# artis-mcrt/artis

Hardware: AMD Instinct MI355X
Metric: packet-steps/sec (higher is better)
Workload: dtype f64

## Files before the change

### artis_amd/build.py

```python
from __future__ import annotations

import fcntl
import os
import shutil
import subprocess

HERE = os.path.dirname(os.path.abspath(__file__))
CSRC = os.path.join(HERE, "csrc")
SO = os.path.join(HERE, "libartis_amd.so")
SOURCES = ["artis_engine.hip", "physics.h", "tables.h", "model_build.h", "spectra.h", "radfield_fit.h", "ion_balance.h",
           "stage_common.h", "stage_spectra.h", "stage_radfield.h", "stage_ionbal.h"]
FLAGS = ["-O3", "--offload-arch=gfx950", "-std=c++17", "-fPIC", "-shared", "-ffp-contract=off", "-munsafe-fp-atomics",
         "-fno-slp-vectorize", "-mllvm", "-disable-machine-licm", "-ldl"]


PRESETS = ("classic", "kilonova_lte", "nltenebular", "christinenonthermal", "nltephotospheric", "nltewithoutnonthermal", "nltenebular_lineest", "kilonova_barnes", "kilonova_wollaeger", "kilonova_gammaproducts",
           "kilonova_gamma_barnes", "kilonova_gamma_wollaeger", "kilonova_gamma_guttman", "kilonova_gamma_grey", "classic_gamma_xcom",
           "kilonova_expopac", "classic_expopac_therm",
           "ci_kilonova", "ci_kilonova_barnes", "ci_kilonova_expopac", "ci_kilonova_xcom", "ci_nebular", "ci_nebular_limitbfest",
           "ci_nltephotospheric", "ci_classic_vpkt", "ci_classic_vpkt_expopac")


def so_path(preset: str = "classic") -> str:
    return SO if preset == "classic" else os.path.join(HERE, f"libartis_amd_{preset}.so")


def needs_build(preset: str = "classic") -> bool:
    so = so_path(preset)
    if not os.path.exists(so):
        return True
    t = os.path.getmtime(so)
    deps = [os.path.join(CSRC, s) for s in SOURCES] + [os.path.join(HERE, "..", "include", h)
                                                        for h in ("artis_amd.h", "artis_options.h")]
# ... 30 lines not shown
```

### artis_amd/csrc/artis_engine.hip

```cpp
#include <hip/hip_runtime.h>
#include <rccl/rccl.h>

#include <dlfcn.h>

#include <cstdio>
#include <cstdlib>
#include <algorithm>
#include <chrono>
#include <cstring>
#include <string>
#include <type_traits>
#include <vector>
#include <cmath>

#include "model_build.h"
#include "physics.h"
#include "radfield_fit.h"
#include "ion_balance.h"
#include "spectra.h"

#include <rocprim/device/device_radix_sort.hpp>

using namespace artis;

// ... 572 lines not shown
    const int src = __ffsll((long long)m) - 1;
    ma_fill_record_wave(env, __builtin_amdgcn_readlane(c, src), __builtin_amdgcn_readlane(ul, src));
    m &= m - 1;
  }
}
__global__ void __launch_bounds__(BLOCK) k_debug_macache(Env env, int c, double *maprocessrates, double *matrans, int32_t *bad) {
  const int ul = blockIdx.x * BLOCK + threadIdx.x;
  if (ul >= env.M.nlevels) return;
  if (ma_resolve(env, c, env.M.level_pack[ul].rec_off) == MA_REC_NONE) return;
  const int b = debug_level_record(env, c, ul, maprocessrates, matrans);
  if (b != 0) atomicAdd(bad, b);
}
__global__ void __launch_bounds__(BLOCK) k_ma_reset(Env env) {
  const int64_t i = (int64_t)blockIdx.x * BLOCK + threadIdx.x;
  const int ncold = env.M.ncold;
  if (i >= fill_count(env) * ncold) return;
  const int c = fill_cell(env, i / ncold);
  env.K.ma_rowtab[(krow(env, c) * ncold) + (i % ncold)] = -1;
}
__global__ void __launch_bounds__(BLOCK) k_mainit(Env env, int64_t nrows) {
  const int64_t i = (int64_t)blockIdx.x * BLOCK + threadIdx.x;
  if (i >= nrows * env.M.nlevels) return;
  populate_mainit(env, i / env.M.nlevels, (int)(i % env.M.nlevels));
}
__global__ void __launch_bounds__(BLOCK) k_cooling_head(Env env) {
  const int64_t i = (int64_t)blockIdx.x * BLOCK + threadIdx.x;
  const int64_t total = fill_count(env) * env.M.nions;
  if (i >= total) return;
  const int c = fill_cell(env, i / env.M.nions);
  const int ui = (int)(i % env.M.nions);
  int k = 0;
  env.K.ion_cooling_C[(krow(env, c) * env.M.nions) + ui] = cooling_ion_head(env, c, ui, &k);
}
__device__ inline double row_shr1(double x) {
  int lo = __double2loint(x), hi = __double2hiint(x);
  lo = __builtin_amdgcn_update_dpp(0, lo, 0x111 , 0xF, 0xF, false);
  hi = __builtin_amdgcn_update_dpp(0, hi, 0x111, 0xF, 0xF, false);
  return __hiloint2double(hi, lo);
}
__global__ void __launch_bounds__(BLOCK) k_cooling_chain(Env env) {
  const int64_t row_id = ((int64_t)blockIdx.x * BLOCK + threadIdx.x) >> 4;
  const int r = threadIdx.x & 15;
  const DevModel &M = env.M;
  const int64_t nchains = fill_count(env) * M.nions;
  const bool valid = row_id < nchains;
  const int c = fill_cell(env, (valid ? row_id : 0) / M.nions);
// ... 2206 lines not shown
  if (const char *b = std::getenv("ARTIS_AMD_SORT_MAXPC_T")) e->sort_maxpc_t = std::max(1, std::atoi(b));
  if (const char *b = std::getenv("ARTIS_AMD_WAVECHUNKS_R")) e->wave_chunks_r = std::atoi(b) != 0;
  if (const char *b = std::getenv("ARTIS_AMD_WAVECHUNKS_T")) e->wave_chunks_t = std::atoi(b) != 0;
  if (const char *b = std::getenv("ARTIS_AMD_CUCHUNKS_T")) e->cu_chunks_t = std::atoi(b) != 0;
  if (const char *b = std::getenv("ARTIS_AMD_CONTLDS")) e->cont_lds = std::atoi(b) != 0;
  if (const char *b = std::getenv("ARTIS_AMD_LINELDS")) e->line_lds = std::atoi(b) != 0;
  if (const char *b = std::getenv("ARTIS_AMD_TILE_ZIGZAG")) e->tile_zigzag = std::atoi(b) != 0;
  if (const char *b = std::getenv("ARTIS_AMD_TILE_ADAPT")) e->tile_adapt = std::atoi(b) != 0;
  if (const char *b = std::getenv("ARTIS_AMD_TILE_BLOCK")) e->tile_block = std::max<int64_t>(0, std::atoll(b));
  if (const char *b = std::getenv("ARTIS_AMD_POOL_KEEP")) e->pool_keep = std::atoi(b) != 0;
  if (const char *b = std::getenv("ARTIS_AMD_MATABLES_LDS")) e->ma_tables_lds = std::atoi(b) != 0;
  if (const char *b = std::getenv("ARTIS_AMD_REFILL")) e->thermal_refill = std::atoi(b) != 0;
  if (const char *b = std::getenv("ARTIS_AMD_SORT_NUMAJOR")) e->sort_numajor = std::atoi(b) != 0;
  if (const char *b = std::getenv("ARTIS_AMD_SORT_CELLSHIFT")) e->sort_cellshift = e->sort_numajor ? std::max(0, std::min(20, std::atoi(b))) : 0;
  if (const char *b = std::getenv("ARTIS_AMD_TQ_LOW")) e->tq_low = std::max(1, std::min(64, std::atoi(b)));
  if (const char *b = std::getenv("ARTIS_AMD_SPARSE_FILL")) e->sparse_fill = std::atoi(b) != 0;
  if (const char *b = std::getenv("ARTIS_AMD_SPARSE_MAX")) e->sparse_max_listed = std::max(0, std::atoi(b));
  {
    const int64_t nrows_ = e->tile_cells;
    Env env0 = make_env(e);
    env0.K = e->K;
    hipLaunchKernelGGL(k_mainit, dim3(nblocks(nrows_ * e->Mh.nlevels)), dim3(BLOCK), 0, nullptr, env0, nrows_);
    HIP_TRY(hipGetLastError());
    HIP_TRY(hipDeviceSynchronize());
  }
  {
    const double mb = pop_scratch_mb();
    const int64_t per = std::max<int64_t>(1, (int64_t)e->Mh.nupcum) * (int64_t)sizeof(double);
    e->pop_batch = std::max<int64_t>(1, std::min<int64_t>(e->tile_cells, (int64_t)(mb * 1048576.) / per));
    HIP_TRY(hipMalloc((void **)&e->d_collexc_terms, (size_t)(e->pop_batch * per) + 64));
  }
  if (const char *b = std::getenv("ARTIS_AMD_THERMAL_BLOCKS")) e->thermal_blocks_per_cu = std::max(1, std::min(ARTIS_THERMAL_WAVES, std::atoi(b)));
  e->trace = std::getenv("ARTIS_AMD_TRACE") != nullptr;
  if (e->trace)
    fprintf(stderr, "[artis_amd] record tiers: static records for %.2f of every ion's levels, %d cold levels, pool of %d slots per resident cell; %d tile(s) of %lld cells, %zu B per cell\n",
            e->ma_hotfrac, e->Mh.ncold, e->Mh.ma_pool_slots, e->ntiles, (long long)e->tile_cells, e->cache_bytes_per_cell);
  if (const char *b = std::getenv("ARTIS_AMD_VPKT_CONTLDS")) e->vpkt_cont_lds = std::atoi(b) != 0;
  if (const char *b = std::getenv("ARTIS_AMD_TILE_PARK")) e->park_tails = std::atoi(b) != 0;
  if (const char *b = std::getenv("ARTIS_AMD_TILE_PARK_AT")) e->park_at = std::max<int64_t>(0, std::atoll(b));
  return ARTIS_OK;
}
}

extern "C" {

void artis_amd_engine_destroy(artis_amd_engine *e) {
// ... 1214 lines not shown
```

### artis_amd/csrc/model_build.h

```cpp
#pragma once
#include <algorithm>
#include <cmath>
#include <cstdlib>
#include <cstring>
#include <vector>

#include "tables.h"

namespace artis {

struct ModelOwned {
  std::vector<double> temperature_grid;
  std::vector<int32_t> level_ion;
  std::vector<LinePack> line_pack;
  std::vector<LevelPack> level_pack;
  std::vector<int32_t> level_upcum_start;
  std::vector<int32_t> alltrans_owner;
  std::vector<int32_t> scanblk_seg0;
  std::vector<uint8_t> scanperm;
  std::vector<MaLongSeg> scansegs, malongsegs;
  std::vector<MaTarget> alltrans_target;
  std::vector<uint16_t> alltrans_tlevel16;
  std::vector<CoolLineRef> coollines;
  std::vector<ContPack> cont_pack;
  std::vector<int32_t> expopac_linestart;
  std::vector<int32_t> upcum_coolslot;
  std::vector<int32_t> level_recomb_start, recomb_lower, recomb_target, recomb_levels, ion_cooltail_start, level_coolhi, ion_guideoff, ion_guideshift;
};

#define ARTIS_MODEL_ARRAYS(X, m)                                                   \
  X(temperature_grid, double, (ARTIS_OPT_TABLESIZE + 1))                           \
  X(elem_nions, int32_t, (m).nelements)                                            \
  X(elem_uniqueionindexstart, int32_t, (m).nelements)                              \
  X(elem_lowest_ionstage, int32_t, (m).nelements)                                  \
  X(elem_anumber, int32_t, (m).nelements)                                          \
  X(ion_element, int32_t, (m).nions)                                               \
  X(ion_nlevels, int32_t, (m).nions)                                               \
  X(ion_nlevels_ionising, int32_t, (m).nions)                                      \
  X(ion_maxrecombininglevel, int32_t, (m).nions)                                   \
  X(ion_uniquelevelindexstart, int32_t, (m).nions)                                 \
  X(ion_coolingoffset, int32_t, (m).nions)                                         \
  X(ion_ncoolingterms, int32_t, (m).nions)                                         \
  X(level_epsilon, double, (m).nlevels)                                            \
  X(level_statweight, float, (m).nlevels)                                          \
  X(level_alltrans_startdown, int32_t, (m).nlevels)                                \
  X(level_ndowntrans, int32_t, (m).nlevels)                                        \
  X(level_nuptrans, int32_t, (m).nlevels)                                          \
  X(level_closestgroundlevelcont, int32_t, (m).nlevels)                            \
  X(level_phixsstart, int32_t, (m).nlevels)                                        \
  X(level_nphixstargets, int32_t, (m).nlevels)                                     \
  X(level_phixstargetstart, int32_t, (m).nlevels)                                  \
  X(level_bflist_start, int32_t, (m).nlevels)                                      \
  X(level_matransblock_start, int32_t, (m).nlevels)                                \
  X(level_ion, int32_t, (m).nlevels)                                               \
  X(level_pack, LevelPack, (m).nlevels)                                            \
  X(level_coolhi, int32_t, (m).nlevels)                                            \
  X(ion_guideoff, int32_t, (m).nions)                                              \
  X(ion_guideshift, int32_t, (m).nions)                                            \
  X(level_upcum_start, int32_t, (m).nlevels)                                       \
  X(alltrans_lineindex, int32_t, (m).nalltrans)                                    \
  X(alltrans_targetlevelindex, int32_t, (m).nalltrans)                             \
  X(alltrans_owner, int32_t, (m).nalltrans)                                        \
  X(scansegs, MaLongSeg, ((m).nscansegs > 0 ? (m).nscansegs : 1))                  \
  X(scanblk_seg0, int32_t, ((m).nscanblk + 1))                                     \
  X(scanperm, uint8_t, ((m).nalltrans > 0 ? (m).nalltrans : 1))                    \
  X(malongsegs, MaLongSeg, ((m).nmalongsegs > 0 ? (m).nmalongsegs : 1))            \
  X(alltrans_target, MaTarget, (m).nalltrans)                                      \
  X(alltrans_tlevel16, uint16_t, (((m).nalltrans + 1) & ~1))  \
  X(coollines, CoolLineRef, ((m).ncoollines > 0 ? (m).ncoollines : 1))             \
  X(alltrans_einstein_A, float, (m).nalltrans)                                     \
  X(alltrans_coll_str, float, (m).nalltrans)                                       \
  X(alltrans_osc_strength, float, (m).nalltrans)                                   \
  X(alltrans_forbidden, uint8_t, (m).nalltrans)                                    \
  X(line_nu, double, (m).nlines)                                                   \
  X(line_pack, LinePack, (m).nlines)                                               \
  X(cont_pack, ContPack, (m).nbfcontinua)                                          \
  X(line_elementindex, int32_t, (m).nlines)                                        \
  X(line_ionindex, int32_t, (m).nlines)                                            \
  X(allphixs, float, ((int64_t)(m).nphixslevels * (m).NPHIXSPOINTS))               \
  X(allphixstargets_levelindex, int32_t, (m).nphixstargets_total)                  \
  X(allphixstargets_probability, double, (m).nphixstargets_total)                  \
  X(allcont_nu_edge, double, (m).nbfcontinua)                                      \
  X(allcont_element, int32_t, (m).nbfcontinua)                                     \
  X(allcont_ion, int32_t, (m).nbfcontinua)                                         \
  X(allcont_level, int32_t, (m).nbfcontinua)                                       \
  X(allcont_phixstargetindex, int32_t, (m).nbfcontinua)                            \
  X(allcont_upperlevel, int32_t, (m).nbfcontinua)                                  \
  X(allcont_uniquelevelindex, int32_t, (m).nbfcontinua)                            \
  X(allcont_groundcontestimindex, int32_t, (m).nbfcontinua)                        \
  X(allcont_probability, double, (m).nbfcontinua)                                  \
// ... 356 lines not shown
  ARTIS_COPY_PTR(coolinglist_type) ARTIS_COPY_PTR(coolinglist_level) ARTIS_COPY_PTR(coolinglist_phixstargetindex)
  ARTIS_COPY_PTR(propcell_nonemptymgi)
#undef ARTIS_COPY_PTR
  v.gridtype = m.gridtype;
  int stride = 1;
  for (int a = 0; a < 3; a++) {
    v.ncoordgrid[a] = m.ncoordgrid[a];
    v.coordstride[a] = stride;
    stride *= m.ncoordgrid[a];
    v.coord_pos_min_tmin[a] = m.coord_pos_min_tmin[a];
  }
  v.ngrid = m.ngrid;
  v.npts_nonempty = m.npts_nonempty;
  v.tmin = m.tmin; v.vmax = m.vmax; v.rmax = m.rmax;
  v.ejecta_kinetic_energy = m.ejecta_kinetic_energy; v.mtot_input = m.mtot_input;
  v.allcont_bfestimindex = m.allcont_bfestimindex;
  v.rho_tmin = m.rho_tmin;
  v.xcom_elem_start = m.xcom_elem_start; v.xcom_energy = m.xcom_energy; v.xcom_sigma = m.xcom_sigma;
  v.nxcom = m.xcom_elem_start ? m.xcom_elem_start[m.nelements] : 0;
  v.detailed_lineindices = m.detailed_lineindices;
  v.detailed_linecount = m.detailed_lineindices ? m.detailed_linecount : 0;
  v.nbfestim = (m.allcont_bfestimindex && m.nbfestim > 0) ? m.nbfestim : m.nbfcontinua;
  v.vpkt = nullptr;
  return v;
}

inline double loggrid_edge(double minvalue, double dlog, double index) { return std::exp(std::log(minvalue) + (index * dlog)); }
inline bool make_vpkt_config(const artis_model &m, VpktConfig &V) {
  std::memset(&V, 0, sizeof(V));
  if (m.vpkt_nobsdirections < 1 || m.vpkt_nobsdirections > VPKT_MAXOBS || !m.vpkt_obsdirs_costheta || !m.vpkt_obsdirs_phi ||
      m.vpkt_nspectraperobsdir < 1 || m.vpkt_nspectraperobsdir > VPKT_MAXSPEC || !m.vpkt_opacityexclusions ||
      m.vpkt_nwavelengthranges < 1 || m.vpkt_nwavelengthranges > VPKT_MAXRANGES || !m.vpkt_numin_input || !m.vpkt_numax_input ||
      m.vpkt_nprocs < 1)
    return false;
  if (m.vpkt_vgrid_on && (m.vpkt_grid_nwavelengthranges < 1 || m.vpkt_grid_nwavelengthranges > VPKT_MAXRANGES || !m.vpkt_nu_grid_min ||
                          !m.vpkt_nu_grid_max))
    return false;
  V.nobsdirections = m.vpkt_nobsdirections;
  V.nspectraperobsdir = m.vpkt_nspectraperobsdir;
  V.nwavelengthranges = m.vpkt_nwavelengthranges;
  V.vgrid_on = m.vpkt_vgrid_on ? 1 : 0;
  V.grid_nwavelengthranges = m.vpkt_vgrid_on ? m.vpkt_grid_nwavelengthranges : 0;
  V.nprocs = m.vpkt_nprocs;
  for (int i = 0; i < V.nobsdirections; i++) {
    const double ct = m.vpkt_obsdirs_costheta[i], ph = m.vpkt_obsdirs_phi[i];
    V.obsdir[i][0] = std::sqrt(1 - (ct * ct)) * std::cos(ph);
// ... 76 lines not shown
```

### artis_amd/csrc/physics.h

```cpp
#pragma once
#include <math.h>
#include <stdint.h>

#include "tables.h"

#if defined(__HIPCC__) && !defined(ARTIS_HOST_EMU)
#define AHD __host__ __device__ inline
#define ANOINLINE static __host__ __device__ __attribute__((noinline))
#else
#define AHD inline
#define ANOINLINE static __attribute__((noinline))
#endif

namespace artis {

constexpr double CLIGHT = 2.99792458e+10;
constexpr double CLIGHT_PROP = CLIGHT;
constexpr double HPLANCK = 6.6260755e-27;
constexpr double PI = 3.14159265358979323846;
constexpr double EV = 1.6021772e-12;
constexpr double SIGMA_T = 6.6524e-25;
constexpr double ME = 9.1093897e-28;
constexpr double MH = 1.67352e-24;
constexpr double MEV = 1.6021772e-6;
constexpr double MSUN = 1.98855e+33;
constexpr double DAY = 86400.;
constexpr double THOMSON_LIMIT = 1e-2;
constexpr double NU_100KEV = 2.41326e+19, NU_1MEV = 2.41326e+20, NU_1P022MEV = 2.46636e+20, NU_1P5MEV = 3.61990e+20;
constexpr double KB = 1.38064852e-16;
constexpr double SAHACONST = 2.0706659e-16;
constexpr double EULERGAMMA = 0.577215664901532860606512090082402431;
constexpr double CLIGHTSQUARED = CLIGHT * CLIGHT;
constexpr double CLIGHTSQUAREDOVERTWOH = CLIGHT * CLIGHT / (2 * HPLANCK);
constexpr double HOVERKB = HPLANCK / KB;
constexpr double HCLIGHTOVERFOURPI = HPLANCK * CLIGHT / (4 * PI);
constexpr double H_ionpot = 13.5979996 * EV;
constexpr double C_0 = 5.465e-11;
constexpr double DBLMAX = 1.7976931348623157e308;
constexpr double DBLMIN = 2.2250738585072014e-308;
constexpr int MA_N = ARTIS_MA_ACTION_COUNT;

#if defined(__HIP_DEVICE_COMPILE__)
typedef unsigned long long stat_t;
#define ARTIS_STAT_ADD(env, i, v) atomicAdd(&(env).stats[(i)], (stat_t)(v))
#ifdef ARTIS_EST_NOADD
#define ARTIS_EST_ADD(ptr, v)                                 \
  do {                                                        \
    const double est_v = (v);                                 \
    if (est_v == 1.2345e-300) unsafeAtomicAdd((ptr), est_v);  \
  } while (0)
#else
#define ARTIS_EST_ADD(ptr, v) unsafeAtomicAdd((ptr), (v))
#endif
#else
typedef unsigned long long stat_t;
#define ARTIS_STAT_ADD(env, i, v) ((env).stats[(i)] += (stat_t)(v))
#define ARTIS_EST_ADD(ptr, v) (*(ptr) += (v))
#endif
#define ARTIS_STAT(env, i) ARTIS_STAT_ADD(env, i, 1)
#if defined(ARTIS_PROFILE) && ARTIS_OPT_VPKT_ON
#error "-DARTIS_PROFILE keeps its phase clocks in the stats slots 48..52, which a VPKT_ON build uses for nvpkt_created / nvpkt_esc_*"
#endif
// ... 102 lines not shown
      }
      vsums[slot] = 0.;
      tags[slot] = c;
    }
  }
  if (tags[slot] == c)
    __hip_atomic_fetch_add((__attribute__((address_space(3))) double *)(env.estcache + slot), v, __ATOMIC_RELAXED, __HIP_MEMORY_SCOPE_WORKGROUP);
  else
    ARTIS_EST_ADD(&global_array[(int64_t)c * env.est_stride], v);
}
#endif

template <typename EnvT>
AHD void scalar_add(const EnvT &env, int idx, double v) {
#if defined(__HIP_DEVICE_COMPILE__)
  if (env.scalars_lds != nullptr) {
    __hip_atomic_fetch_add((__attribute__((address_space(3))) double *)(env.scalars_lds + idx), v, __ATOMIC_RELAXED, __HIP_MEMORY_SCOPE_WORKGROUP);
    return;
  }
#endif
  ARTIS_EST_ADD(&env.E.scalars[idx], v);
}

AHD double pow2(double x) { return x * x; }
AHD double pow3(double x) { return x * x * x; }
AHD double dmin(double a, double b) { return (b < a) ? b : a; }
AHD double dmax(double a, double b) { return (a < b) ? b : a; }
AHD double dclamp(double v, double lo, double hi) { return (v < lo) ? lo : ((hi < v) ? hi : v); }

struct Env {
  DevModel M;
  DevCells C;
  DevCache K;
  DevStep S;
  DevEst E;
  PktStore P;
  stat_t *stats;
  double *gamma_ws;
  int32_t *gamma_gi;
  int32_t *gamma_n;
  int32_t *errflag;
  const int32_t *krow_tab;
  int32_t tile_all;
  int32_t tile_lo, tile_hi;
  const int32_t *fill_cells;
  int32_t nfill;
  double *collexc_terms;
  int32_t cont_in_lds;
// ... 611 lines not shown
  const int gridsize = ARTIS_OPT_TABLESIZE + 1;
  int index = (int)(log(T / ARTIS_OPT_MINTEMP) / M.T_step_log) + 1;
  if (index < 0) index = 0;
  if (index > gridsize) index = gridsize;
  while (index > 0 && M.temperature_grid[index - 1] > T) index--;
  while (index < gridsize && M.temperature_grid[index] <= T) index++;
  return index;
}
AHD double lerp_or_last(const DevModel &M, const double *table, int ul, int t, float T) {
  const double *row = table + ((int64_t)(M.level_bflist_start[ul] + t) * ARTIS_OPT_TABLESIZE);
  const int up = temperature_upperindex(M, T);
  if (up == 0) return row[0];
  if (up < ARTIS_OPT_TABLESIZE) {
    const double T_lower = M.temperature_grid[up - 1];
    const double T_upper = M.temperature_grid[up];
    const double f_lower = row[up - 1];
    const double f_upper = row[up];
    return (f_lower + ((f_upper - f_lower) / (T_upper - T_lower) * (T - T_lower)));
  }
  return row[ARTIS_OPT_TABLESIZE - 1];
}

AHD double gaunt_factor(int stage) { return stage == 1 ? 0.1 : (stage == 2 ? 0.2 : 0.3); }
AHD double rad_deexc(double epsilon_trans, float A_ul, double gu, double gl, double n_u, double n_l, double t) {
  const double nu_trans = epsilon_trans / HPLANCK;
  const double B_ul = CLIGHTSQUAREDOVERTWOH / pow3(nu_trans) * A_ul;
  const double B_lu = gu / gl * B_ul;
  const double tau = ((B_lu * n_l) - (B_ul * n_u)) * HCLIGHTOVERFOURPI * t;
  if (tau > 1e-100) {
    const double beta = 1.0 / tau * (-expm1(-tau));
    return A_ul * beta;
  }
  return A_ul;
}
#if ARTIS_OPT_DETAILED_LINE_ESTIMATORS_ON
AHD int jblueindex(const DevModel &M, int lineindex) {
  int low = 0, high = M.detailed_linecount - 1;
  while (low <= high) {
    const int mid = low + ((high - low) / 2);
    if (M.detailed_lineindices[mid] < lineindex) low = mid + 1;
    else if (M.detailed_lineindices[mid] > lineindex) high = mid - 1;
    else return mid;
  }
  return -1;
}
AHD void update_lineestimator(const Env &env, int c, int lineindex, double increment) {
  const int jb = jblueindex(env.M, lineindex);
  if (jb >= 0) {
    const int64_t o = ((int64_t)c * env.M.detailed_linecount) + jb;
    ARTIS_EST_ADD(&env.E.Jb_lu_raw[o], increment);
    ARTIS_EST_ADD(&env.E.Jb_lu_contribcount[o], 1.);
  }
}
#endif
AHD double rad_exc(const Env &env, int c, double gu, double A, double epsilon_trans, double n_l, double n_u, double gl, double t,
                   int alltransindex = -1) {
  const double nu_trans = epsilon_trans / HPLANCK;
  const double B_ul = CLIGHTSQUAREDOVERTWOH / pow3(nu_trans) * A;
  const double B_lu = gu / gl * B_ul;
  const double tau = ((B_lu * n_l) - (B_ul * n_u)) * HCLIGHTOVERFOURPI * t;
  if (tau > 1e-100) {
    const double beta = 1.0 / tau * (-expm1(-tau));
    const double R_over_J = n_l > 0. ? (B_lu - (B_ul * n_u / n_l)) * beta : B_lu * beta;
#if ARTIS_OPT_DETAILED_LINE_ESTIMATORS_ON
    if (alltransindex >= 0) {
      const int jb = jblueindex(env.M, env.M.alltrans_lineindex[alltransindex]);
      if (jb >= 0) return R_over_J * env.C.Jb_lu_normed[((int64_t)c * env.M.detailed_linecount) + jb];
    }
#endif
    return R_over_J * radfield(env, nu_trans, c);
  }
  return 0.;
}
AHD double rad_recomb(const DevModel &M, float T_e, float cnne, int element, int upperion, int lowerlevel, int t) {
  return cnne * lerp_or_last(M, M.spontrecombcoeffs, lstart(M, element, upperion - 1) + lowerlevel, t, T_e);
}
AHD double col_recomb(const DevModel &M, float T_e, float cnne, int element, int upperion, int lower, int t, double epsilon_trans) {
  const int ul = lstart(M, element, upperion - 1) + lower;
  const double gl = statw(M, ul);
  const double g = gaunt_factor(ionstage(M, element, upperion - 1));
  const double sigma_bf = (phixs_table(M, ul)[0] * phixs_probability(M, ul, t));
  const double gu = statw(M, lstart(M, element, upperion) + phixs_upperlevel(M, ul, t));
  return cnne * cnne * SAHACONST * gl / gu * 1.55e13 * g * sigma_bf * KB / T_e / epsilon_trans;
}
AHD double col_ion(const DevModel &M, float T_e, float cnne, int element, int ion, int lower, int t, double epsilon_trans) {
  const int ul = lstart(M, element, ion) + lower;
  const double g = gaunt_factor(ionstage(M, element, ion));
  const double fac1 = epsilon_trans / KB / T_e;
  const double sigma_bf = phixs_table(M, ul)[0] * phixs_probability(M, ul, t);
  return cnne * 1.55e13 * pow((double)T_e, -0.5) * g * sigma_bf * exp(-fac1) / fac1;
}
AHD double col_deexc(const DevModel &M, float T_e, float cnne, double epsilon_trans, double gu, double gl, int ati) {
  const float cs = M.alltrans_coll_str[ati];
  if (cs < 0) {
    if (!M.alltrans_forbidden[ati]) {
      const double f = M.alltrans_osc_strength[ati];
      const double eoverkt = epsilon_trans / (KB * T_e);
      const double g_bar = 0.2;
      const double gauntfac = (eoverkt > 0.33421) ? g_bar : 0.276 * exp(eoverkt) * (-EULERGAMMA - log(eoverkt));
      const double g_ratio = gl / gu;
      return C_0 * 14.51039491 * cnne * sqrtf(T_e) * f * pow2(H_ionpot / epsilon_trans) * eoverkt * g_ratio * gauntfac;
    }
    return cnne * 8.629e-6 * 0.01 * gl / sqrtf(T_e);
  }
  return cnne * 8.629e-6 * (double)cs / gu / sqrtf(T_e);
}
AHD double col_exc(const DevModel &M, float T_e, float cnne, double epsilon_trans, double gu, double gl, int ati) {
  const float cs = M.alltrans_coll_str[ati];
  const double eoverkt = epsilon_trans / (KB * T_e);
  if (cs < 0) {
    if (!M.alltrans_forbidden[ati]) {
      const double f = M.alltrans_osc_strength[ati];
      const double g_bar = 0.2;
      const double ex = exp(eoverkt);
      const double Gamma = dmax(g_bar, 0.276 * ex * (-EULERGAMMA - log(eoverkt)));
      return C_0 * cnne * sqrtf(T_e) * 14.51039491 * f * pow2(H_ionpot / epsilon_trans) * eoverkt / ex * Gamma;
    }
    return cnne * 8.629e-6 * 0.01 * exp(-eoverkt) * gu / sqrtf(T_e);
  }
  return cnne * 8.629e-6 * (double)cs * exp(-eoverkt) / gl / sqrtf(T_e);
}


AHD void populate_levelpop(const Env &env, int c, int ul) {
  const DevModel &M = env.M;
  if (env.C.levelpops) {
    env.K.levelpops[(krow(env, c) * M.nlevels) + ul] = env.C.levelpops[((int64_t)c * M.nlevels) + ul];
    return;
  }
  const int ui = M.level_ion[ul];
  const int element = M.ion_element[ui];
  const int ion = ui - M.elem_uniqueionindexstart[element];
  const int start = M.ion_uniquelevelindexstart[ui];
  const double nnground = groundlevelpop(env, c, element, ion);
  double nn;
  if (ul == start) {
    nn = nnground;
  } else {
    const float T_exc = ARTIS_OPT_LTEPOP_EXCITATION_USE_TJ ? env.C.TJ[c] : env.C.Te[c];
    const double E_aboveground = eps(M, ul) - eps(M, start);
    nn = (nnground * statw(M, ul) / statw(M, start) * exp(-E_aboveground / KB / T_exc));
  }
  if (nn < ARTIS_OPT_MINPOP) nn = (env.C.elem_massfracs[((int64_t)c * M.nelements) + element] > 0) ? ARTIS_OPT_MINPOP : 0.;
// ... 212 lines not shown
  }
  return !bad;
}
AHD double nt_excitation_ratecoeff(const DevCells &C, int c, int lowerlevel, int upperlevel, int alltransindex) {
  if (!ARTIS_OPT_NT_EXCITATION_ON) return 0.;
  if (lowerlevel >= ARTIS_OPT_NTEXCITATION_MAXNLEVELS_LOWER) return 0.;
  if (upperlevel >= ARTIS_OPT_NTEXCITATION_MAXNLEVELS_UPPER) return 0.;
  const int64_t base = (int64_t)c * C.nt_excitations_stored;
  const int32_t *ati = C.nt_exc_alltransindex + base;
  const int n = C.nt_exc_count[c];
  int lo = 0, hi = n;
  while (lo < hi) {
    const int mid = lo + ((hi - lo) / 2);
    if (ati[mid] < alltransindex) lo = mid + 1; else hi = mid;
  }
  if (lo == n || ati[lo] != alltransindex) return 0.;
  return C.nt_exc_ratecoeffperdeposition[base + lo] * C.nt_deposition_rate_density[c];
}
#endif

struct MaTransTerms {
  int ul, i;
  bool isdown;
  LevelPack lpk;
  double v0, v1, v2;
  double kterm;
};
template <bool COOLING_ONLY_IF_COLD = false>
AHD MaTransTerms matrans_terms(const Env &env, int c, int ati) {
  const DevModel &M = env.M;
  MaTransTerms r;
  r.ul = M.alltrans_owner[ati];
  r.lpk = M.level_pack[r.ul];
  const int ul = r.ul;
  if (COOLING_ONLY_IF_COLD && r.lpk.rec_off < 0) {
    const int i = ati - r.lpk.alltrans_startdown;
    r.isdown = i < r.lpk.ndown;
    r.i = r.isdown ? i : i - r.lpk.ndown;
    r.v0 = r.v1 = r.v2 = r.kterm = 0.;
    if (!r.isdown) {
      const int tul = M.ion_uniquelevelindexstart[M.level_ion[ul]] + M.alltrans_targetlevelindex[ati];
      const double e_trans = eps(M, tul) - eps(M, ul);
      const double Cc = col_exc(M, env.C.Te[c], clumpednne(env.C, c), e_trans, statw(M, tul), statw(M, ul), ati);
      r.kterm = env.K.levelpops[(krow(env, c) * M.nlevels) + ul] * Cc * e_trans;
    }
    return r;
  }
  const int start = M.ion_uniquelevelindexstart[M.level_ion[ul]];
  const double *pops = env.K.levelpops + (krow(env, c) * M.nlevels);
  const float T_e = env.C.Te[c];
  const float cnne = clumpednne(env.C, c);
  const double e_cur = eps(M, ul);
  const double g_cur = statw(M, ul);
  const double nnlevel = pops[ul];
  const int i = ati - r.lpk.alltrans_startdown;
  const int tul = start + M.alltrans_targetlevelindex[ati];
  r.isdown = i < r.lpk.ndown;
  r.kterm = 0.;
  if (r.isdown) {
    r.i = i;
    const float A_ul = M.alltrans_einstein_A[ati];
    const double e_target = eps(M, tul);
    const double e_trans = e_cur - e_target;
    const double g_low = statw(M, tul);
    const double R = rad_deexc(e_trans, A_ul, g_cur, g_low, nnlevel, pops[tul], env.S.mid);
    const double Cc = col_deexc(M, T_e, cnne, e_trans, g_cur, g_low, ati);
    r.v0 = R * e_trans;
    r.v1 = Cc * e_trans;
    r.v2 = (R + Cc) * e_target;
  } else {
    r.i = i - r.lpk.ndown;
    const double e_trans = eps(M, tul) - e_cur;
    const double g_up = statw(M, tul);
    const double R = rad_exc(env, c, g_up, M.alltrans_einstein_A[ati], e_trans, nnlevel, pops[tul], g_cur, env.S.mid, ati);
    const double Cc = col_exc(M, T_e, cnne, e_trans, g_up, g_cur, ati);
#if ARTIS_OPT_NT_ON
    const double NT = nt_excitation_ratecoeff(env.C, c, ul - start, M.alltrans_targetlevelindex[ati], ati);
#else
    const double NT = 0.;
#endif
    r.v0 = (R + Cc + NT) * e_cur;
    r.v1 = 0.;
    r.v2 = 0.;
    r.kterm = nnlevel * Cc * e_trans;
  }
  return r;
}
AHD int32_t ma_rowtab_load(const int32_t *p) {
#if defined(__HIP_DEVICE_COMPILE__)
  return __hip_atomic_load(p, __ATOMIC_RELAXED, __HIP_MEMORY_SCOPE_AGENT);
#else
  return *p;
#endif
}
AHD void ma_rowtab_acquire(const Env &env, int32_t v) {
#if defined(__HIP_DEVICE_COMPILE__)
  if (env.ma_concurrent_fill != 0 && v >= 0) __builtin_amdgcn_fence(__ATOMIC_ACQUIRE, "agent");
#else
  (void)env;
  (void)v;
#endif
}
constexpr int MA_REC_NONE = -1;
template <bool COLD = true>
AHD int ma_resolve(const Env &env, int c, int rec_off) {
  if (!COLD) return rec_off;
  if (__builtin_expect(rec_off >= 0, 1)) return rec_off;
// ... 4126 lines not shown
```

### artis_amd/csrc/tables.h

```cpp
#pragma once
#include <stdint.h>

#include "../../include/artis_amd.h"
#include "../../include/artis_options.h"

namespace artis {

struct alignas(16) LinePack {
  int32_t lower;
  int32_t upper;
  float B_ul;
  float B_lu;
};

struct alignas(16) LevelPack {
  int32_t rec_off;
  int32_t alltrans_startdown;
  int32_t ndown;
  int32_t nup;
};
struct alignas(32) ContPack {
  double nu_edge;
  double probability;
  int32_t xs_off;
  int32_t gi;
  int32_t pad[2];
};
struct alignas(16) MaTarget {
  int32_t rec, ats, level;
  uint32_t ndnu;
};
constexpr int MATGT_MAX_NTRANS = 1 << 16;
static_assert(sizeof(MaTarget) == 16, "transition target size");
struct alignas(16) U4 {
  uint32_t w[4];
};
constexpr int MAREC_ALIGN = 4;
constexpr int MAPOOL_UNIT = 8;
constexpr int MAREC_PER = 7;
constexpr int MAREC_QUAD = 4;
constexpr int MAREC_RATE_SLOTS = 5;
enum { MADIR_DOWN = 0, MADIR_UP = 1, MADIR_RAD = 2, MADIR_COOL = 3 };
constexpr int marec_lines(int n) { return (n + MAREC_PER - 1) / MAREC_PER; }
constexpr int marec_rest(int n) { return n > MAREC_PER ? marec_lines(n) - 1 : 0; }
constexpr int marec_slot(int d, int l, int nd, int nu) {
  return (d < MADIR_COOL && l == 0)
             ? 1 + d
             : (d == MADIR_DOWN ? MAREC_QUAD + (l - 1)
                                : (d == MADIR_UP ? MAREC_QUAD + marec_rest(nd) + (l - 1)
                                                 : (d == MADIR_RAD ? MAREC_QUAD + marec_rest(nd) + marec_rest(nu) + (l - 1)
                                                                   : MAREC_QUAD + (2 * marec_rest(nd)) + marec_rest(nu) + l)));
}
constexpr int marec_rates_slot(int nd, int nu) { return MAREC_QUAD + (2 * marec_rest(nd)) + marec_rest(nu) + marec_lines(nu); }
constexpr int marec_fine_dirslots(int n) { return (marec_lines(n) + 1) / 2; }
constexpr int marec_fine_slot0(int nd, int nu) { return marec_rates_slot(nd, nu) + MAREC_RATE_SLOTS; }
constexpr int marec_fine_byte0(int d, int l, int nd, int nu) {
// ... 51 lines not shown
  const int32_t *xcom_elem_start;
  const double *xcom_energy, *xcom_sigma;
  int32_t nxcom;
  const int32_t *detailed_lineindices;
  int32_t detailed_linecount;
  const VpktConfig *vpkt;
  const int32_t *ion_element, *ion_nlevels, *ion_nlevels_ionising, *ion_maxrecombininglevel, *ion_uniquelevelindexstart,
      *ion_coolingoffset, *ion_ncoolingterms;
  const double *level_epsilon;
  const float *level_statweight;
  const int32_t *level_alltrans_startdown, *level_ndowntrans, *level_nuptrans, *level_closestgroundlevelcont, *level_phixsstart,
      *level_nphixstargets, *level_phixstargetstart, *level_bflist_start, *level_matransblock_start;
  const int32_t *level_ion;
  const LevelPack *level_pack;
  const int32_t *level_upcum_start;
  const int32_t *alltrans_lineindex, *alltrans_targetlevelindex;
  const int32_t *alltrans_owner;
  const MaLongSeg *scansegs;
  const int32_t *scanblk_seg0;
  int32_t nscansegs, nscanblk;
  const uint8_t *scanperm;
  const MaLongSeg *malongsegs;
  int32_t nmalongsegs;
  const MaTarget *alltrans_target;
  const uint16_t *alltrans_tlevel16;
  const CoolLineRef *coollines;
  int32_t ncoollines;
  const float *alltrans_einstein_A, *alltrans_coll_str, *alltrans_osc_strength;
  const uint8_t *alltrans_forbidden;
  const double *line_nu;
  const LinePack *line_pack;
  const ContPack *cont_pack;
  const int32_t *line_elementindex, *line_ionindex;
  const float *allphixs;
  const int32_t *allphixstargets_levelindex;
  const double *allphixstargets_probability;
  const double *allcont_nu_edge;
  const int32_t *allcont_element, *allcont_ion, *allcont_level, *allcont_phixstargetindex, *allcont_upperlevel,
      *allcont_uniquelevelindex, *allcont_groundcontestimindex;
  const double *allcont_probability;
  const double *groundcont_nu_edge;
  const double *spontrecombcoeffs, *corrphotoioncoeffs, *bfcooling_coeffs;
  const uint8_t *coolinglist_type;
  const int32_t *coolinglist_level, *coolinglist_phixstargetindex;

  int32_t gridtype, ncoordgrid[3], coordstride[3], ngrid, npts_nonempty;
// ... 133 lines not shown
```

Measured before the change: 1.375 billion.

## Precompute per-transition constants into a packed TransConst table

Adds a 96-byte TransConst record per transition. A one-time kernel fills it at init with energies, frequency, Einstein B coefficients, statistical weights, flags and indices. matrans_terms now reads this single record instead of gathering level_pack, epsilon, statweight, coll_str and other arrays, and recomputing B coefficients and pow3 per call. The aim is fewer scattered loads and less arithmetic in the macro-atom transition rate evaluation. The cost is extra device memory and a wider per-transition load, and the lower-level energy is now used in place of the current level energy in some terms.

Result: no change. 1.380 billion, median of 6 (+0.3%).

```diff
diff --git a/artis_amd/build.py b/artis_amd/build.py
--- a/artis_amd/build.py
+++ b/artis_amd/build.py
@@ -8,7 +8,7 @@
 HERE = os.path.dirname(os.path.abspath(__file__))
 CSRC = os.path.join(HERE, "csrc")
 SO = os.path.join(HERE, "libartis_amd.so")
-SOURCES = ["artis_engine.hip", "physics.h", "tables.h", "model_build.h", "spectra.h", "radfield_fit.h", "ion_balance.h",
+SOURCES = ["artis_engine.hip", "physics.h", "constants.h", "transconst.h", "tables.h", "model_build.h", "spectra.h", "radfield_fit.h", "ion_balance.h",
            "stage_common.h", "stage_spectra.h", "stage_radfield.h", "stage_ionbal.h"]
 FLAGS = ["-O3", "--offload-arch=gfx950", "-std=c++17", "-fPIC", "-shared", "-ffp-contract=off", "-munsafe-fp-atomics",
          "-fno-slp-vectorize", "-mllvm", "-disable-machine-licm", "-ldl"]
diff --git a/artis_amd/csrc/artis_engine.hip b/artis_amd/csrc/artis_engine.hip
--- a/artis_amd/csrc/artis_engine.hip
+++ b/artis_amd/csrc/artis_engine.hip
@@ -618,6 +618,11 @@
   const int64_t i = (int64_t)blockIdx.x * BLOCK + threadIdx.x;
   if (i >= nrows * env.M.nlevels) return;
   populate_mainit(env, i / env.M.nlevels, (int)(i % env.M.nlevels));
+}
+__global__ void __launch_bounds__(BLOCK) k_transconst(DevModel M, TransConst *out) {
+  const int ati = blockIdx.x * BLOCK + threadIdx.x;
+  if (ati >= M.nalltrans) return;
+  out[ati] = transconst_of(M, ati);
 }
 __global__ void __launch_bounds__(BLOCK) k_cooling_head(Env env) {
   const int64_t i = (int64_t)blockIdx.x * BLOCK + threadIdx.x;
@@ -2870,6 +2875,10 @@
     env0.K = e->K;
     hipLaunchKernelGGL(k_mainit, dim3(nblocks(nrows_ * e->Mh.nlevels)), dim3(BLOCK), 0, nullptr, env0, nrows_);
     HIP_TRY(hipGetLastError());
+    if (e->Mh.nalltrans > 0) {
+      hipLaunchKernelGGL(k_transconst, dim3(nblocks(e->Mh.nalltrans)), dim3(BLOCK), 0, nullptr, e->M, const_cast<TransConst *>(e->M.transconst));
+      HIP_TRY(hipGetLastError());
+    }
     HIP_TRY(hipDeviceSynchronize());
   }
   {
diff --git a/artis_amd/csrc/constants.h b/artis_amd/csrc/constants.h
--- /dev/null
+++ b/artis_amd/csrc/constants.h
@@ -0,0 +1,41 @@
+#pragma once
+
+#if defined(__HIPCC__) && !defined(ARTIS_HOST_EMU)
+#define AHD __host__ __device__ inline
+#define ANOINLINE static __host__ __device__ __attribute__((noinline))
+#else
+#define AHD inline
+#define ANOINLINE static __attribute__((noinline))
+#endif
+
+namespace artis {
+
+constexpr double CLIGHT = 2.99792458e+10;
+constexpr double CLIGHT_PROP = CLIGHT;
+constexpr double HPLANCK = 6.6260755e-27;
+constexpr double PI = 3.14159265358979323846;
+constexpr double EV = 1.6021772e-12;
+constexpr double SIGMA_T = 6.6524e-25;
+constexpr double ME = 9.1093897e-28;
+constexpr double MH = 1.67352e-24;
+constexpr double MEV = 1.6021772e-6;
+constexpr double MSUN = 1.98855e+33;
+constexpr double DAY = 86400.;
+constexpr double THOMSON_LIMIT = 1e-2;
+constexpr double NU_100KEV = 2.41326e+19, NU_1MEV = 2.41326e+20, NU_1P022MEV = 2.46636e+20, NU_1P5MEV = 3.61990e+20;
+constexpr double KB = 1.38064852e-16;
+constexpr double SAHACONST = 2.0706659e-16;
+constexpr double EULERGAMMA = 0.577215664901532860606512090082402431;
+constexpr double CLIGHTSQUARED = CLIGHT * CLIGHT;
+constexpr double CLIGHTSQUAREDOVERTWOH = CLIGHT * CLIGHT / (2 * HPLANCK);
+constexpr double HOVERKB = HPLANCK / KB;
+constexpr double HCLIGHTOVERFOURPI = HPLANCK * CLIGHT / (4 * PI);
+constexpr double H_ionpot = 13.5979996 * EV;
+constexpr double C_0 = 5.465e-11;
+constexpr double DBLMAX = 1.7976931348623157e308;
+constexpr double DBLMIN = 2.2250738585072014e-308;
+
+AHD double pow2(double x) { return x * x; }
+AHD double pow3(double x) { return x * x * x; }
+
+}
diff --git a/artis_amd/csrc/model_build.h b/artis_amd/csrc/model_build.h
--- a/artis_amd/csrc/model_build.h
+++ b/artis_amd/csrc/model_build.h
@@ -6,6 +6,7 @@
 #include <vector>
 
 #include "tables.h"
+#include "transconst.h"
 
 namespace artis {
 
@@ -20,6 +21,7 @@
   std::vector<uint8_t> scanperm;
   std::vector<MaLongSeg> scansegs, malongsegs;
   std::vector<MaTarget> alltrans_target;
+  std::vector<TransConst> transconst;
   std::vector<uint16_t> alltrans_tlevel16;
   std::vector<CoolLineRef> coollines;
   std::vector<ContPack> cont_pack;
@@ -66,6 +68,7 @@
   X(scanperm, uint8_t, ((m).nalltrans > 0 ? (m).nalltrans : 1))                    \
   X(malongsegs, MaLongSeg, ((m).nmalongsegs > 0 ? (m).nmalongsegs : 1))            \
   X(alltrans_target, MaTarget, (m).nalltrans)                                      \
+  X(transconst, TransConst, ((m).nalltrans > 0 ? (m).nalltrans : 1))               \
   X(alltrans_tlevel16, uint16_t, (((m).nalltrans + 1) & ~1))  \
   X(coollines, CoolLineRef, ((m).ncoollines > 0 ? (m).ncoollines : 1))             \
   X(alltrans_einstein_A, float, (m).nalltrans)                                     \
@@ -468,6 +471,11 @@
   v.detailed_linecount = m.detailed_lineindices ? m.detailed_linecount : 0;
   v.nbfestim = (m.allcont_bfestimindex && m.nbfestim > 0) ? m.nbfestim : m.nbfcontinua;
   v.vpkt = nullptr;
+  own.transconst.assign((size_t)(m.nalltrans > 0 ? m.nalltrans : 1), TransConst{});
+  v.transconst = own.transconst.data();
+#if defined(ARTIS_HOST_EMU)
+  for (int ati = 0; ati < m.nalltrans; ati++) own.transconst[ati] = transconst_of(v, ati);
+#endif
   return v;
 }
 
diff --git a/artis_amd/csrc/physics.h b/artis_amd/csrc/physics.h
--- a/artis_amd/csrc/physics.h
+++ b/artis_amd/csrc/physics.h
@@ -3,41 +3,11 @@
 #include <stdint.h>
 
 #include "tables.h"
-
-#if defined(__HIPCC__) && !defined(ARTIS_HOST_EMU)
-#define AHD __host__ __device__ inline
-#define ANOINLINE static __host__ __device__ __attribute__((noinline))
-#else
-#define AHD inline
-#define ANOINLINE static __attribute__((noinline))
-#endif
+#include "constants.h"
+#include "transconst.h"
 
 namespace artis {
 
-constexpr double CLIGHT = 2.99792458e+10;
-constexpr double CLIGHT_PROP = CLIGHT;
-constexpr double HPLANCK = 6.6260755e-27;
-constexpr double PI = 3.14159265358979323846;
-constexpr double EV = 1.6021772e-12;
-constexpr double SIGMA_T = 6.6524e-25;
-constexpr double ME = 9.1093897e-28;
-constexpr double MH = 1.67352e-24;
-constexpr double MEV = 1.6021772e-6;
-constexpr double MSUN = 1.98855e+33;
-constexpr double DAY = 86400.;
-constexpr double THOMSON_LIMIT = 1e-2;
-constexpr double NU_100KEV = 2.41326e+19, NU_1MEV = 2.41326e+20, NU_1P022MEV = 2.46636e+20, NU_1P5MEV = 3.61990e+20;
-constexpr double KB = 1.38064852e-16;
-constexpr double SAHACONST = 2.0706659e-16;
-constexpr double EULERGAMMA = 0.577215664901532860606512090082402431;
-constexpr double CLIGHTSQUARED = CLIGHT * CLIGHT;
-constexpr double CLIGHTSQUAREDOVERTWOH = CLIGHT * CLIGHT / (2 * HPLANCK);
-constexpr double HOVERKB = HPLANCK / KB;
-constexpr double HCLIGHTOVERFOURPI = HPLANCK * CLIGHT / (4 * PI);
-constexpr double H_ionpot = 13.5979996 * EV;
-constexpr double C_0 = 5.465e-11;
-constexpr double DBLMAX = 1.7976931348623157e308;
-constexpr double DBLMIN = 2.2250738585072014e-308;
 constexpr int MA_N = ARTIS_MA_ACTION_COUNT;
 
 #if defined(__HIP_DEVICE_COMPILE__)
@@ -186,8 +156,6 @@
   ARTIS_EST_ADD(&env.E.scalars[idx], v);
 }
 
-AHD double pow2(double x) { return x * x; }
-AHD double pow3(double x) { return x * x * x; }
 AHD double dmin(double a, double b) { return (b < a) ? b : a; }
 AHD double dmax(double a, double b) { return (a < b) ? b : a; }
 AHD double dclamp(double v, double lo, double hi) { return (v < lo) ? lo : ((hi < v) ? hi : v); }
@@ -845,17 +813,6 @@
 }
 
 AHD double gaunt_factor(int stage) { return stage == 1 ? 0.1 : (stage == 2 ? 0.2 : 0.3); }
-AHD double rad_deexc(double epsilon_trans, float A_ul, double gu, double gl, double n_u, double n_l, double t) {
-  const double nu_trans = epsilon_trans / HPLANCK;
-  const double B_ul = CLIGHTSQUAREDOVERTWOH / pow3(nu_trans) * A_ul;
-  const double B_lu = gu / gl * B_ul;
-  const double tau = ((B_lu * n_l) - (B_ul * n_u)) * HCLIGHTOVERFOURPI * t;
-  if (tau > 1e-100) {
-    const double beta = 1.0 / tau * (-expm1(-tau));
-    return A_ul * beta;
-  }
-  return A_ul;
-}
 #if ARTIS_OPT_DETAILED_LINE_ESTIMATORS_ON
 AHD int jblueindex(const DevModel &M, int lineindex) {
   int low = 0, high = M.detailed_linecount - 1;
@@ -876,25 +833,6 @@
   }
 }
 #endif
-AHD double rad_exc(const Env &env, int c, double gu, double A, double epsilon_trans, double n_l, double n_u, double gl, double t,
-                   int alltransindex = -1) {
-  const double nu_trans = epsilon_trans / HPLANCK;
-  const double B_ul = CLIGHTSQUAREDOVERTWOH / pow3(nu_trans) * A;
-  const double B_lu = gu / gl * B_ul;
-  const double tau = ((B_lu * n_l) - (B_ul * n_u)) * HCLIGHTOVERFOURPI * t;
-  if (tau > 1e-100) {
-    const double beta = 1.0 / tau * (-expm1(-tau));
-    const double R_over_J = n_l > 0. ? (B_lu - (B_ul * n_u / n_l)) * beta : B_lu * beta;
-#if ARTIS_OPT_DETAILED_LINE_ESTIMATORS_ON
-    if (alltransindex >= 0) {
-      const int jb = jblueindex(env.M, env.M.alltrans_lineindex[alltransindex]);
-      if (jb >= 0) return R_over_J * env.C.Jb_lu_normed[((int64_t)c * env.M.detailed_linecount) + jb];
-    }
-#endif
-    return R_over_J * radfield(env, nu_trans, c);
-  }
-  return 0.;
-}
 AHD double rad_recomb(const DevModel &M, float T_e, float cnne, int element, int upperion, int lowerlevel, int t) {
   return cnne * lerp_or_last(M, M.spontrecombcoeffs, lstart(M, element, upperion - 1) + lowerlevel, t, T_e);
 }
@@ -913,35 +851,32 @@
   const double sigma_bf = phixs_table(M, ul)[0] * phixs_probability(M, ul, t);
   return cnne * 1.55e13 * pow((double)T_e, -0.5) * g * sigma_bf * exp(-fac1) / fac1;
 }
-AHD double col_deexc(const DevModel &M, float T_e, float cnne, double epsilon_trans, double gu, double gl, int ati) {
-  const float cs = M.alltrans_coll_str[ati];
+AHD double col_deexc_k(const TransConst &k, float cnne, double eoverkt, float sqrt_Te) {
+  const float cs = k.coll_str;
   if (cs < 0) {
-    if (!M.alltrans_forbidden[ati]) {
-      const double f = M.alltrans_osc_strength[ati];
-      const double eoverkt = epsilon_trans / (KB * T_e);
+    if (!(k.flags & TRANSCONST_FORBIDDEN)) {
+      const double f = k.osc_strength;
       const double g_bar = 0.2;
       const double gauntfac = (eoverkt > 0.33421) ? g_bar : 0.276 * exp(eoverkt) * (-EULERGAMMA - log(eoverkt));
-      const double g_ratio = gl / gu;
-      return C_0 * 14.51039491 * cnne * sqrtf(T_e) * f * pow2(H_ionpot / epsilon_trans) * eoverkt * g_ratio * gauntfac;
-    }
-    return cnne * 8.629e-6 * 0.01 * gl / sqrtf(T_e);
-  }
-  return cnne * 8.629e-6 * (double)cs / gu / sqrtf(T_e);
-}
-AHD double col_exc(const DevModel &M, float T_e, float cnne, double epsilon_trans, double gu, double gl, int ati) {
-  const float cs = M.alltrans_coll_str[ati];
-  const double eoverkt = epsilon_trans / (KB * T_e);
+      return C_0 * 14.51039491 * cnne * sqrt_Te * f * k.hion2 * eoverkt * k.g_ratio * gauntfac;
+    }
+    return cnne * 8.629e-6 * 0.01 * (double)k.g_lower / sqrt_Te;
+  }
+  return cnne * 8.629e-6 * (double)cs / (double)k.g_upper / sqrt_Te;
+}
+AHD double col_exc_k(const TransConst &k, float cnne, double eoverkt, float sqrt_Te) {
+  const float cs = k.coll_str;
   if (cs < 0) {
-    if (!M.alltrans_forbidden[ati]) {
-      const double f = M.alltrans_osc_strength[ati];
+    if (!(k.flags & TRANSCONST_FORBIDDEN)) {
+      const double f = k.osc_strength;
       const double g_bar = 0.2;
       const double ex = exp(eoverkt);
       const double Gamma = dmax(g_bar, 0.276 * ex * (-EULERGAMMA - log(eoverkt)));
-      return C_0 * cnne * sqrtf(T_e) * 14.51039491 * f * pow2(H_ionpot / epsilon_trans) * eoverkt / ex * Gamma;
-    }
-    return cnne * 8.629e-6 * 0.01 * exp(-eoverkt) * gu / sqrtf(T_e);
-  }
-  return cnne * 8.629e-6 * (double)cs * exp(-eoverkt) / gl / sqrtf(T_e);
+      return C_0 * cnne * sqrt_Te * 14.51039491 * f * k.hion2 * eoverkt / ex * Gamma;
+    }
+    return cnne * 8.629e-6 * 0.01 * exp(-eoverkt) * (double)k.g_upper / sqrt_Te;
+  }
+  return cnne * 8.629e-6 * (double)cs * exp(-eoverkt) / (double)k.g_lower / sqrt_Te;
 }
 
 
@@ -1200,67 +1135,57 @@
 struct MaTransTerms {
   int ul, i;
   bool isdown;
-  LevelPack lpk;
   double v0, v1, v2;
   double kterm;
 };
 template <bool COOLING_ONLY_IF_COLD = false>
 AHD MaTransTerms matrans_terms(const Env &env, int c, int ati) {
-  const DevModel &M = env.M;
+  const TransConst k = env.M.transconst[ati];
   MaTransTerms r;
-  r.ul = M.alltrans_owner[ati];
-  r.lpk = M.level_pack[r.ul];
-  const int ul = r.ul;
-  if (COOLING_ONLY_IF_COLD && r.lpk.rec_off < 0) {
-    const int i = ati - r.lpk.alltrans_startdown;
-    r.isdown = i < r.lpk.ndown;
-    r.i = r.isdown ? i : i - r.lpk.ndown;
-    r.v0 = r.v1 = r.v2 = r.kterm = 0.;
-    if (!r.isdown) {
-      const int tul = M.ion_uniquelevelindexstart[M.level_ion[ul]] + M.alltrans_targetlevelindex[ati];
-      const double e_trans = eps(M, tul) - eps(M, ul);
-      const double Cc = col_exc(M, env.C.Te[c], clumpednne(env.C, c), e_trans, statw(M, tul), statw(M, ul), ati);
-      r.kterm = env.K.levelpops[(krow(env, c) * M.nlevels) + ul] * Cc * e_trans;
-    }
-    return r;
-  }
-  const int start = M.ion_uniquelevelindexstart[M.level_ion[ul]];
-  const double *pops = env.K.levelpops + (krow(env, c) * M.nlevels);
+  r.ul = k.ul;
+  r.i = k.i;
+  r.isdown = (k.flags & TRANSCONST_DOWN) != 0;
+  r.v0 = r.v1 = r.v2 = r.kterm = 0.;
+  const double *pops = env.K.levelpops + (krow(env, c) * env.M.nlevels);
   const float T_e = env.C.Te[c];
   const float cnne = clumpednne(env.C, c);
-  const double e_cur = eps(M, ul);
-  const double g_cur = statw(M, ul);
-  const double nnlevel = pops[ul];
-  const int i = ati - r.lpk.alltrans_startdown;
-  const int tul = start + M.alltrans_targetlevelindex[ati];
-  r.isdown = i < r.lpk.ndown;
-  r.kterm = 0.;
+  const double eoverkt = k.e_trans / (KB * T_e);
+  const float sqrt_Te = sqrtf(T_e);
+  if (COOLING_ONLY_IF_COLD && (k.flags & TRANSCONST_COLD)) {
+    if (!r.isdown) r.kterm = pops[k.ul] * col_exc_k(k, cnne, eoverkt, sqrt_Te) * k.e_trans;
+    return r;
+  }
+  const double n_u = pops[r.isdown ? k.ul : k.tul], n_l = pops[r.isdown ? k.tul : k.ul];
+  const double tau = ((k.B_lu * n_l) - (k.B_ul * n_u)) * HCLIGHTOVERFOURPI * env.S.mid;
+  const bool thick = tau > 1e-100;
+  double beta = 0.;
+  if (thick) beta = 1.0 / tau * (-expm1(-tau));
   if (r.isdown) {
-    r.i = i;
-    const float A_ul = M.alltrans_einstein_A[ati];
-    const double e_target = eps(M, tul);
-    const double e_trans = e_cur - e_target;
-    const double g_low = statw(M, tul);
-    const double R = rad_deexc(e_trans, A_ul, g_cur, g_low, nnlevel, pops[tul], env.S.mid);
-    const double Cc = col_deexc(M, T_e, cnne, e_trans, g_cur, g_low, ati);
-    r.v0 = R * e_trans;
-    r.v1 = Cc * e_trans;
-    r.v2 = (R + Cc) * e_target;
+    const double R = thick ? k.A_ul * beta : (double)k.A_ul;
+    const double Cc = col_deexc_k(k, cnne, eoverkt, sqrt_Te);
+    r.v0 = R * k.e_trans;
+    r.v1 = Cc * k.e_trans;
+    r.v2 = (R + Cc) * k.e_lower;
   } else {
-    r.i = i - r.lpk.ndown;
-    const double e_trans = eps(M, tul) - e_cur;
-    const double g_up = statw(M, tul);
-    const double R = rad_exc(env, c, g_up, M.alltrans_einstein_A[ati], e_trans, nnlevel, pops[tul], g_cur, env.S.mid, ati);
-    const double Cc = col_exc(M, T_e, cnne, e_trans, g_up, g_cur, ati);
+    double R = 0.;
+    if (thick) {
+      const double R_over_J = n_l > 0. ? (k.B_lu - (k.B_ul * n_u / n_l)) * beta : k.B_lu * beta;
+#if ARTIS_OPT_DETAILED_LINE_ESTIMATORS_ON
+      const int jb = jblueindex(env.M, env.M.alltrans_lineindex[ati]);
+      if (jb >= 0) R = R_over_J * env.C.Jb_lu_normed[((int64_t)c * env.M.detailed_linecount) + jb];
+      else
+#endif
+      R = R_over_J * radfield(env, k.nu_trans, c);
+    }
+    const double Cc = col_exc_k(k, cnne, eoverkt, sqrt_Te);
 #if ARTIS_OPT_NT_ON
-    const double NT = nt_excitation_ratecoeff(env.C, c, ul - start, M.alltrans_targetlevelindex[ati], ati);
+    const int start = env.M.ion_uniquelevelindexstart[env.M.level_ion[k.ul]];
+    const double NT = nt_excitation_ratecoeff(env.C, c, k.ul - start, env.M.alltrans_targetlevelindex[ati], ati);
 #else
     const double NT = 0.;
 #endif
-    r.v0 = (R + Cc + NT) * e_cur;
-    r.v1 = 0.;
-    r.v2 = 0.;
-    r.kterm = nnlevel * Cc * e_trans;
+    r.v0 = (R + Cc + NT) * k.e_lower;
+    r.kterm = n_l * Cc * k.e_trans;
   }
   return r;
 }
diff --git a/artis_amd/csrc/tables.h b/artis_amd/csrc/tables.h
--- a/artis_amd/csrc/tables.h
+++ b/artis_amd/csrc/tables.h
@@ -32,6 +32,17 @@
 };
 constexpr int MATGT_MAX_NTRANS = 1 << 16;
 static_assert(sizeof(MaTarget) == 16, "transition target size");
+struct alignas(32) TransConst {
+  double e_trans, nu_trans, B_ul, B_lu;
+  double hion2, e_lower, g_ratio;
+  float A_ul, coll_str;
+  float osc_strength, g_upper, g_lower;
+  int32_t ul, tul, i, flags, pad;
+};
+static_assert(sizeof(TransConst) == 96, "transition constants: three 32-byte pieces");
+constexpr int32_t TRANSCONST_DOWN = 1;
+constexpr int32_t TRANSCONST_FORBIDDEN = 2;
+constexpr int32_t TRANSCONST_COLD = 4;
 struct alignas(16) U4 {
   uint32_t w[4];
 };
@@ -129,6 +140,7 @@
   const uint8_t *scanperm;
   const MaLongSeg *malongsegs;
   int32_t nmalongsegs;
+  const TransConst *transconst;
   const MaTarget *alltrans_target;
   const uint16_t *alltrans_tlevel16;
   const CoolLineRef *coollines;
diff --git a/artis_amd/csrc/transconst.h b/artis_amd/csrc/transconst.h
--- /dev/null
+++ b/artis_amd/csrc/transconst.h
@@ -0,0 +1,41 @@
+#pragma once
+#include "constants.h"
+#include "tables.h"
+
+namespace artis {
+
+AHD TransConst transconst_of(const DevModel &M, int ati) {
+  TransConst k;
+  const int ul = M.alltrans_owner[ati];
+  const LevelPack lpk = M.level_pack[ul];
+  const int tul = M.ion_uniquelevelindexstart[M.level_ion[ul]] + M.alltrans_targetlevelindex[ati];
+  const int i = ati - lpk.alltrans_startdown;
+  const bool isdown = i < lpk.ndown;
+  const int upper = isdown ? ul : tul, lower = isdown ? tul : ul;
+  const float A_ul = M.alltrans_einstein_A[ati];
+  const double gu = M.level_statweight[upper], gl = M.level_statweight[lower];
+  const double epsilon_trans = M.level_epsilon[upper] - M.level_epsilon[lower];
+  const double nu_trans = epsilon_trans / HPLANCK;
+  const double B_ul = CLIGHTSQUAREDOVERTWOH / pow3(nu_trans) * A_ul;
+  const double B_lu = gu / gl * B_ul;
+  k.e_trans = epsilon_trans;
+  k.nu_trans = nu_trans;
+  k.B_ul = B_ul;
+  k.B_lu = B_lu;
+  k.hion2 = pow2(H_ionpot / epsilon_trans);
+  k.e_lower = M.level_epsilon[lower];
+  k.g_ratio = gl / gu;
+  k.A_ul = A_ul;
+  k.coll_str = M.alltrans_coll_str[ati];
+  k.osc_strength = M.alltrans_osc_strength[ati];
+  k.g_upper = M.level_statweight[upper];
+  k.g_lower = M.level_statweight[lower];
+  k.ul = ul;
+  k.tul = tul;
+  k.i = isdown ? i : i - lpk.ndown;
+  k.flags = (isdown ? TRANSCONST_DOWN : 0) | (M.alltrans_forbidden[ati] ? TRANSCONST_FORBIDDEN : 0) | (lpk.rec_off < 0 ? TRANSCONST_COLD : 0);
+  k.pad = 0;
+  return k;
+}
+
+}
```
